# MannLabs/alphadia

Measured on AMD Instinct MI355X. Metric: precursors scored/sec, higher is better.
Workload: dtype f32/f64; 1 GPU; 1000000-precursor predicted library x 3 candidates vs 2h synthetic Thermo-style DIA run (4800 cycles x 61 spectra); BASELINE configs[2] on one GPU; precursors_total=1000000, candidates_total=3000000, candidates_per_gpu=3000000, cycles=4800, parallelism=single GPU, rccl_ranks_seen=1, priming_steps_before_warmup=4

## Files before the change

### alphadia_amd/_abi.py

```python

from __future__ import annotations

import ctypes as C

import numpy as np

NUM_FEATURES = 46
FLAG_SKIP = 1

_f32p = C.POINTER(C.c_float)
_f64p = C.POINTER(C.c_double)
_i64p = C.POINTER(C.c_int64)
_u32p = C.POINTER(C.c_uint32)
_u8p = C.POINTER(C.c_uint8)


class AlphaRaw(C.Structure):
    _fields_ = [
        ("cycle", _f64p),
        ("cycle_len", C.c_int32),
        ("cycle_scans", C.c_int32),
        ("rt_values", _f32p),
        ("n_spectra", C.c_int64),
        ("mobility_values", _f32p),
# ... 123 lines not shown
        ("fragment_precursor_idx", _u32p),
        ("fragment_rank", _u8p),
        ("fragment_mz_library", _f32p),
        ("fragment_mz", _f32p),
        ("fragment_mz_observed", _f32p),
        ("fragment_height", _f32p),
        ("fragment_intensity", _f32p),
        ("fragment_mass_error", _f32p),
        ("fragment_correlation", _f32p),
        ("fragment_position", _u8p),
        ("fragment_number", _u8p),
        ("fragment_type", _u8p),
        ("fragment_charge", _u8p),
        ("fragment_loss_type", _u8p),
    ]


COMPACT_ROW_FIELDS = [("row", np.uint32), ("precursor_idx", np.uint32), ("rank", np.uint8)]
COMPACT_SLOT_FIELDS = [
    ("fragment_row", np.uint32), ("fragment_precursor_idx", np.uint32), ("fragment_rank", np.uint8),
    ("fragment_mz_library", np.float32), ("fragment_mz", np.float32), ("fragment_mz_observed", np.float32),
    ("fragment_height", np.float32), ("fragment_intensity", np.float32), ("fragment_mass_error", np.float32),
    ("fragment_correlation", np.float32), ("fragment_position", np.uint8), ("fragment_number", np.uint8),
    ("fragment_type", np.uint8), ("fragment_charge", np.uint8), ("fragment_loss_type", np.uint8),
]


OUTPUT_FIELDS = [
    ("valid", np.uint8, 1),
    ("precursor_idx", np.uint32, 1),
# ... 568 lines not shown
    "adh_calibrate_staged_fragments": [C.c_void_p, C.POINTER(LoessModel), C.POINTER(C.c_double)],
    "adh_stage_fragments_columns": [C.c_void_p, C.POINTER(Fragments), C.POINTER(LoessModel), C.POINTER(C.c_double)],
    "adh_staged_fragments_read": [C.c_void_p, C.c_int32, C.c_void_p, C.c_int64],
}


N_PLAN_CLASSES = 37
N_GENERIC_GROUPS = 3
PLAN_PROTOTYPES = {
    "adh_plan_class_counts": [C.c_void_p, C.POINTER(C.c_int64), C.c_int32],
    "adh_generic_launch_stats": [C.c_void_p, C.POINTER(C.c_int64), C.c_int32],
}


def declare(lib) -> None:
    for name, argtypes in {**RESIDENT_PROTOTYPES, **STAGE_PART_PROTOTYPES, **APPEND_PROTOTYPES, **QUANT_PROTOTYPES,
                           **PG_PROTOTYPES, **PFDR_PROTOTYPES, **TL_PROTOTYPES, **MBR_PROTOTYPES, **STAGE_LIB_PROTOTYPES, **PLAN_PROTOTYPES}.items():
        fn = getattr(lib, name)
        fn.argtypes = argtypes
        fn.restype = C.c_int
```

### alphadia_amd/csrc/adh_copyout.hip

```cpp

__global__ void adh_slot_count_kernel(const uint16_t *__restrict__ lib_slot, int64_t row0, int64_t n, int top_k,
                                      uint32_t *__restrict__ cnt) {
    const int64_t i = (int64_t)blockIdx.x * blockDim.x + threadIdx.x;
    if (i > n) return;
    uint32_t k = 0;
    if (i < n) {
        const uint16_t *s = lib_slot + (row0 + i) * (int64_t)top_k;
        while (k < (uint32_t)top_k && s[k]) ++k;
    }
    cnt[i] = k;
}

#include "adh_fill_host.h"

struct PadLayout {
    size_t per_row, total;
    PadLayout(int64_t n, int top_k, int64_t n_chunks)
        : per_row(4 + (size_t)top_k * 22), total(base(n, n_chunks + 1, 4 + (size_t)top_k * 22) + 64) {}
    size_t base(int64_t a, int64_t ci) const { return base(a, ci, per_row); }
    static size_t base(int64_t a, int64_t ci, size_t per_row_) {
        return ((size_t)a * per_row_ + ((size_t)(a / kAnchorRows) + (size_t)ci) * 8 + (size_t)ci * 1024 + 255) & ~(size_t)255;
    }
};

__global__ void adh_pad_pack_kernel(DevOut t, int64_t row0, int64_t n, int top_k, unsigned char *__restrict__ block,
                                    uint32_t *__restrict__ total) {
    const int64_t id = (int64_t)blockIdx.x * blockDim.x + threadIdx.x;
    const uint32_t *off = reinterpret_cast<const uint32_t *>(block);
// ... 165 lines not shown
        const uint32_t a = (uint32_t)o, k = (uint32_t)o1 - a;
        if ((uint32_t)s >= k) continue;
        const int64_t r = row0 + i, src = r * (int64_t)top_k + s;
        const size_t dst = (size_t)a + (size_t)s;
        s_slot[dst] = t.fragment_lib_slot[src];
        reinterpret_cast<float *>(block + L.s_f[0])[dst] = t.fragment_mz_observed[src];
        reinterpret_cast<float *>(block + L.s_f[1])[dst] = t.fragment_height[src];
        reinterpret_cast<float *>(block + L.s_f[2])[dst] = t.fragment_intensity[src];
        reinterpret_cast<float *>(block + L.s_f[3])[dst] = t.fragment_mass_error[src];
        reinterpret_cast<float *>(block + L.s_f[4])[dst] = t.fragment_correlation[src];
    }
}

namespace {
void cop_copy_stripe(const unsigned char *block, int64_t cnt_r, int64_t cnt_s, int64_t base_r, int64_t base_s,
                     adh_compact_output_t *out, int w, int T, const adh_candidates_t *c, const LibRec *lib) {
    const CopBlock L((uint64_t)cnt_r, (uint64_t)cnt_s);
    const int64_t lo = cnt_r * w / T, hi = cnt_r * (w + 1) / T;
    if (hi <= lo) return;
    const uint32_t *rows = reinterpret_cast<const uint32_t *>(block + L.row);
    const uint8_t *cnt = block + L.cnt;
    int64_t s_lo = 0;
    for (int64_t j = 0; j < lo; ++j) s_lo += cnt[j];
    memcpy(out->row + base_r + lo, rows + lo, (size_t)(hi - lo) * 4);
    const float *fb = reinterpret_cast<const float *>(block + L.feat);
    for (int k = 0; k < ADH_NUM_FEATURES; ++k)
        memcpy(out->features + (size_t)k * (size_t)out->rows_capacity + (size_t)(base_r + lo),
               fb + (size_t)k * (size_t)cnt_r + (size_t)lo, (size_t)(hi - lo) * 4);
    const uint16_t *slot = reinterpret_cast<const uint16_t *>(block + L.s_slot);
    int64_t d = base_s + s_lo, at = s_lo;
    for (int64_t j = lo; j < hi; ++j) {
        const uint32_t r = rows[j];
        const uint32_t p = c->precursor_idx[r];
        const uint8_t rk = c->rank ? c->rank[r] : (uint8_t)0;
        out->precursor_idx[base_r + j] = p;
        out->rank[base_r + j] = rk;
        const LibRec *base = lib + c->frag_start_idx[r];
        const int k = (int)cnt[j];
        for (int q = 0; q < k; ++q, ++d, ++at) {
            const LibRec &l = base[slot[at] - 1];
            out->fragment_row[d] = r;
            out->fragment_precursor_idx[d] = p;
            out->fragment_rank[d] = rk;
            out->fragment_mz_library[d] = l.mz_library;
            out->fragment_mz[d] = l.mz;
            out->fragment_position[d] = l.position;
// ... 540 lines not shown
        if (!handoff.wait_for(n_chunks - 1))
            return fail(ADH_ERR_HIP, std::string("scoring pipeline (compacted copy-out): ") + hipGetErrorString(handoff.error));
        for (int64_t ci = 0; ci < n_chunks; ++ci) stripe(ci, T);
        team.join_all();
        if (trace.timing)
            fprintf(stderr, "[adh]   compacted copy-out: host team done %.2f ms after the call began (%d threads)\n", trace.since(), T);
        if (trace.timing && sparse)
            fprintf(stderr, "[adh]   sparse-slot wire: %llu filled slots, %llu intensity words and %llu correlation words sent\n",
                    (unsigned long long)wire_slots, (unsigned long long)wire_nz_i, (unsigned long long)wire_nz_c);
        return ADH_OK;
    }
};

struct OperatorCopyOut : CopyOut {
    adh_compact_output_t *const cop;
    const CopLayout lay;
    const int T;
    int started = 0;
    unsigned char *dev_blocks = nullptr, *stage = nullptr;
    std::vector<int64_t> base_r, base_s, cnt_r, cnt_s;
    bool overflow = false;
    BlockHandoff handoff;
    HandoffTeam team{handoff};
    OperatorCopyOut(const CopyOut &call, adh_compact_output_t *cop_)
        : CopyOut(call), cop(cop_), lay(n, top_k, n_chunks), T(host_threads_for(n)), base_r((size_t)n_chunks + 1, 0),
          base_s((size_t)n_chunks + 1, 0), cnt_r((size_t)n_chunks, 0), cnt_s((size_t)n_chunks, 0),
          handoff(n_chunks, h->device) {}

    void advise_huge_pages() const {
        auto advise = [](void *p, size_t bytes) {
            const uintptr_t lo = ((uintptr_t)p + (2u << 20) - 1) & ~(uintptr_t)((2u << 20) - 1);
            const uintptr_t hi = ((uintptr_t)p + bytes) & ~(uintptr_t)((2u << 20) - 1);
            if (hi > lo) (void)madvise((void *)lo, hi - lo, MADV_HUGEPAGE);
        };
        const size_t rc_ = (size_t)cop->rows_capacity, sc_ = (size_t)cop->slots_capacity;
        advise(cop->features, rc_ * ADH_NUM_FEATURES * 4);
        advise(cop->row, rc_ * 4), advise(cop->precursor_idx, rc_ * 4);
        void *const s4[] = {cop->fragment_row, cop->fragment_precursor_idx, cop->fragment_mz_library, cop->fragment_mz,
                            cop->fragment_mz_observed, cop->fragment_height, cop->fragment_intensity,
                            cop->fragment_mass_error, cop->fragment_correlation};
        for (void *p4 : s4) advise(p4, sc_ * 4);
        void *const s1[] = {cop->fragment_rank, cop->fragment_position, cop->fragment_number, cop->fragment_type,
                            cop->fragment_charge, cop->fragment_loss_type};
        for (void *p1 : s1) advise(p1, sc_);
    }
    int prepare() override {
        if (!compact_output_complete(cop)) return fail(ADH_ERR_INVALID_ARGUMENT, "compact output buffer is NULL");
        advise_huge_pages();
        const size_t cnt_bytes = (size_t)(n + n_chunks) * 8;
        int rc = grow_device(&h->cop_cnt, &h->cop_cnt_bytes, cnt_bytes, cnt_bytes / 8);
        if (rc == ADH_OK) rc = grow_scan_scratch<uint64_t>(&h->cop_scan, &h->cop_scan_bytes, longest_chunk() + 1, h->stream);
        if (rc == ADH_OK) rc = grow_pinned(&h->cop_stage, &h->cop_stage_bytes, lay.total, lay.total / 8);
        if (rc != ADH_OK) return rc;
        if (n_chunks > 4096) return fail(ADH_ERR_UNSUPPORTED, "compact output: more than 4096 chunks");
        if (!h->cop_tot_pinned) HIP_TRY(hipHostMalloc((void **)&h->cop_tot_pinned, 4096 * 8, hipHostMallocDefault));
        rc = grow_device(&h->cop_dev, &h->cop_dev_bytes, lay.total, lay.total / 8 + 4096);
        if (rc != ADH_OK) return rc;
        stage = static_cast<unsigned char *>(h->cop_stage), dev_blocks = static_cast<unsigned char *>(h->cop_dev);
        handoff.landed = [this](int64_t ci) {
            const uint64_t tot = h->cop_tot_pinned[ci];
            base_r[(size_t)ci + 1] = base_r[(size_t)ci] + (int64_t)(tot >> 32);
            base_s[(size_t)ci + 1] = base_s[(size_t)ci] + (int64_t)(tot & 0xFFFFFFFFull);
            if (base_r[(size_t)ci + 1] > cop->rows_capacity || base_s[(size_t)ci + 1] > cop->slots_capacity)
                overflow = true;
            cnt_r[(size_t)ci] = overflow ? 0 : (int64_t)(tot >> 32);
            cnt_s[(size_t)ci] = overflow ? 0 : (int64_t)(tot & 0xFFFFFFFFull);
            if (trace.timing)
                fprintf(stderr, "[adh]   compact chunk %lld: %lld rows, %lld slots on the host %.2f ms after the call began\n",
                        (long long)ci, (long long)(tot >> 32), (long long)(tot & 0xFFFFFFFFull), trace.since());
        };
        return ADH_OK;
    }
    void stripe(int64_t ci, int w) {
        if (cnt_r[(size_t)ci] == 0 && cnt_s[(size_t)ci] == 0) return;
        cop_copy_stripe(stage + lay.base(cut[(size_t)ci], ci), cnt_r[(size_t)ci], cnt_s[(size_t)ci], base_r[(size_t)ci],
                        base_s[(size_t)ci], cop, w, T, c, h->h_lib.data());
    }
    void start_team() override {
        started = start_handoff_team(team, T, n_chunks, [this](int64_t ci, int w) { stripe(ci, w); });
    }
    int pack(int64_t ci) override {
        const int64_t a = cut[(size_t)ci], nr = cut[(size_t)ci + 1] - a;
        hipStream_t sk = h->stream;
        uint64_t *off = static_cast<uint64_t *>(h->cop_cnt) + a + ci;
        hipLaunchKernelGGL(adh_cop_count_kernel, dim3((unsigned)((nr + 256) / 256)), dim3(256), 0, sk, dev.valid,
                           dev.fragment_lib_slot, a, nr, top_k, off);
        size_t scan_bytes = h->cop_scan_bytes;
        HIP_TRY(hipcub::DeviceScan::ExclusiveSum(h->cop_scan, scan_bytes, off, off, (int)(nr + 1), sk));
        hipLaunchKernelGGL(adh_cop_pack_kernel, dim3((unsigned)std::min<int64_t>((nr * top_k + 255) / 256, 8192)), dim3(256), 0,
                           sk, dev, h->cs.d, h->d_lib, a, nr, top_k, off, dev_blocks + lay.base(a, ci), h->cop_tot_pinned + ci);
        HIP_TRY(hipGetLastError());
// ... 9 lines not shown
    }
    int copy_out(int64_t ci) override {
        return ci > 0 ? send(ci - 1) : ADH_OK;
    }
    int flush() override { return send(n_chunks - 1); }
    int finish() override {
        if (!handoff.wait_for(n_chunks - 1))
            return fail(ADH_ERR_HIP, std::string("scoring pipeline (compact copy-out): ") + hipGetErrorString(handoff.error));
        team.join_all();
        for (int64_t ci = 0; ci < n_chunks; ++ci)
            for (int w = started; w < T; ++w) stripe(ci, w);
        if (trace.timing)
            fprintf(stderr, "[adh]   compact: host team done %.2f ms after the call began (%d threads)\n", trace.since(), T);
        cop->n_rows = base_r[(size_t)n_chunks];
        cop->n_slots = base_s[(size_t)n_chunks];
        if (overflow) {
            (void)hipStreamSynchronize(h->stream);
            (void)hipStreamSynchronize(h->stream_out);
            tables_stand = true;
            return fail(ADH_ERR_INVALID_ARGUMENT, "compact output: rows_capacity / slots_capacity too small (n_rows / n_slots say what is needed)");
        }
        return ADH_OK;
    }
};

}
```

### alphadia_amd/csrc/adh_score_host.hip

```cpp

namespace {

int comm_wait_slot(adh_handle *h, int slot);
int comm_gather_slot(adh_handle *h, int slot);

struct OutFieldDesc {
    const char *name;
    size_t member;
    int per_row;
    int elem;
    bool wire;
    bool optional;
};

const OutFieldDesc kOutFields[] = {
    {"valid", offsetof(adh_output_t, valid), 1, 1, true, false},
    {"features", offsetof(adh_output_t, features), ADH_NUM_FEATURES, 4, true, false},
    {"fragment_mz_observed", offsetof(adh_output_t, fragment_mz_observed), -1, 4, true, false},
    {"fragment_height", offsetof(adh_output_t, fragment_height), -1, 4, true, false},
    {"fragment_intensity", offsetof(adh_output_t, fragment_intensity), -1, 4, true, false},
    {"fragment_mass_error", offsetof(adh_output_t, fragment_mass_error), -1, 4, true, false},
    {"fragment_correlation", offsetof(adh_output_t, fragment_correlation), -1, 4, true, false},
    {"fragment_lib_slot", offsetof(adh_output_t, fragment_lib_slot), -1, 2, true, true},
    {"precursor_idx", offsetof(adh_output_t, precursor_idx), 1, 4, false, false},
// ... 1056 lines not shown
        for (std::vector<hipEvent_t> *list : {&events, &aux}) {
            h->free_events.insert(h->free_events.end(), list->begin(), list->end());
            list->clear();
        }
        if (!ok) {
            (void)hipDeviceSynchronize();
            (void)hipGetLastError();
            h->last_tables = -1;
            h->last_rows = 0;
            tab.partial = false;
        }
    }
};

int score_pipeline(adh_handle_t *h, const adh_candidates_t *c, const adh_scoring_config_t *cfg, adh_output_t *out,
                   adh_compact_output_t *cop, bool resident = false) {
    if (!h || !c || !cfg || !out) return fail(ADH_ERR_INVALID_ARGUMENT, "NULL argument");
    if (out->n != c->n) return fail(ADH_ERR_INVALID_ARGUMENT, "output rows != candidates");
    int rc = check_candidate_args(h, c);
    if (rc == ADH_OK) rc = check_score_args(h, cfg, out);
    if (rc != ADH_OK) return rc;
    for (int i = 0; i < kNumOutFields && !cop && !resident; ++i)
        if (!kOutFields[i].optional && *out_member(out, kOutFields[i]) == nullptr)
            return fail(ADH_ERR_INVALID_ARGUMENT, "output buffer is NULL");
    HIP_TRY(hipSetDevice(h->device));
    PipelineTrace trace;
    const int64_t n = c->n;
    const int top_k = out->top_k;
    h->plan = Plan();
    h->cands_uploaded = false;
    h->acc_live = false;
// ... 45 lines not shown
    }
    const std::vector<int64_t> cut = chunk_cuts(n, h->tims_staged, max_rows, compact_wanted);
    const int64_t n_chunks = (int64_t)cut.size() - 1;
    const bool compact = compact_wanted && n_chunks <= 4096;
    adh_output_t dev_k = dev;
    if ((rebuild || cop || resident) && !getenv("ADH_DEBUG_WRITE_ALL")) {
        for (int i = 0; i < kNumOutFields; ++i) {
            const OutFieldDesc &f = kOutFields[i];
            if (!f.wire && f.member != offsetof(adh_output_t, stat_matched_peaks)) *out_member(&dev_k, f) = nullptr;
        }
        tab.partial = true;
    }
    const CopyOut call(h, c, dev, cut, chunk_done, tot_ready, trace);
    std::unique_ptr<CopyOut> copy_out;
    if (resident) copy_out.reset(new CopyOut(call));
    else if (cop) copy_out.reset(new OperatorCopyOut(call, cop));
    else if (compact) copy_out.reset(new PackedCopyOut(call, out));
    else copy_out.reset(new PlainCopyOut(call, out, rebuild));
    rc = copy_out->prepare();
    if (rc != ADH_OK) return rc;
    trace.t_1 = trace.now();
    trace.mark_start(si);
    rc = cand_upload_range(h, c, 0, cut[1], si);
    if (rc == ADH_OK) rc = plan_enqueue(h, h->slots[0], cfg, 0, cut[1], si);
    if (rc == ADH_OK && n_chunks > 1) rc = cand_upload_range(h, c, cut[1], cut[2], si);
    if (rc != ADH_OK) return rc;
    copy_out->start_team();
    for (int64_t ci = 0; ci < n_chunks; ++ci) {
        const int64_t a = cut[(size_t)ci], b = cut[(size_t)ci + 1];
        const int ps = (int)(ci & 1);
        if (ci + 1 < n_chunks) {
// ... 30 lines not shown
    if (e != hipSuccess) return fail(ADH_ERR_HIP, std::string("scoring pipeline: ") + hipGetErrorString(e));
    trace.report(cut, chunk_done, compact);
    unwind.ok = true;
    h->tables_current = true;
    return ADH_OK;
}
}

int adh_score_candidates(adh_handle_t *h, const adh_candidates_t *c, const adh_scoring_config_t *cfg,
                         adh_output_t *out) {
    return score_pipeline(h, c, cfg, out, nullptr);
}

int adh_score_candidates_compact(adh_handle_t *h, const adh_candidates_t *c, const adh_scoring_config_t *cfg,
                                 adh_compact_output_t *cop) {
    if (!h || !c || !cfg || !cop) return fail(ADH_ERR_INVALID_ARGUMENT, "NULL argument");
    if (cop->top_k <= 0 || cop->rows_capacity < 0 || cop->slots_capacity < 0)
        return fail(ADH_ERR_INVALID_ARGUMENT, "compact output: top_k / capacities");
    if (cop->top_k > 255)
        return fail(ADH_ERR_INVALID_ARGUMENT, "compact output: top_k above 255");
    if (h->h_lib.size() != (size_t)h->n_lib)
        return fail(ADH_ERR_NOT_STAGED, "compact output: no host copy of the staged library");
    adh_output_t shape{};
    shape.n = c->n;
    shape.top_k = cop->top_k;
    return score_pipeline(h, c, cfg, &shape, cop);
}

int adh_table_layout(int64_t rows, int32_t top_k, int32_t capacity, adh_table_field_t *fields, int32_t *n_fields,
                     uint64_t *total_bytes, uint64_t *wire_bytes) {
    if (rows < 0 || top_k <= 0 || !n_fields) return fail(ADH_ERR_INVALID_ARGUMENT, "adh_table_layout: bad argument");
    *n_fields = kNumOutFields;
    size_t wire = 0;
    const size_t total = layout_tables(nullptr, rows, top_k, nullptr, &wire);
    if (total_bytes) *total_bytes = total;
    if (wire_bytes) *wire_bytes = wire;
    if (!fields) return ADH_OK;
    if (capacity < kNumOutFields) return fail(ADH_ERR_INVALID_ARGUMENT, "adh_table_layout: field array too short");
    size_t off = 0;
    for (int i = 0; i < kNumOutFields; ++i) {
        const OutFieldDesc &f = kOutFields[i];
// ... 278 lines not shown
```

### alphadia_amd/runtime.py

```python

from __future__ import annotations

import ctypes as C
import os

import numpy as np

from alphadia_amd import _abi

_HERE = os.path.dirname(os.path.abspath(__file__))
LIB_PATH = os.environ.get("ADH_LIB_PATH") or os.path.join(_HERE, "libalphadia_hip.so")

EXPORTED_SYMBOLS = [
    "adh_last_error",
    "adh_device_count",
    "adh_create",
    "adh_destroy",
    "adh_stage_alpharaw",
    "adh_stage_timstof",
    "adh_stage_fragments",
    "adh_score_candidates",
    "adh_score_candidates_compact",
    "adh_host_take_objects",
    "adh_trim_device_cache",
    "adh_host_threads",
    "adh_chunk_cuts",
    "adh_upload_candidates",
    "adh_score_uploaded",
    "adh_get_stream",
    "adh_synchronize",
    "adh_kernel_time_ms",
    "adh_fragcomp",
    "adh_fragcomp_stats",
    "adh_fragcomp_frames",
    "adh_select_candidates",
    "adh_select_time_ms",
    "adh_transpose_timstof",
# ... 106 lines not shown


_PROCESS_T0 = _process_start_time()


def _attempt_lower_bound() -> float:
    if os.environ.get("ADH_RUN_NONCE"):
        return _PROCESS_T0 - float(os.environ.get("ADH_RENDEZVOUS_STAGGER_S", "600"))
    return min(_process_start_time(os.getppid()), _PROCESS_T0)


class HipBackendError(RuntimeError):
    pass


def _load():
    if not os.path.exists(LIB_PATH):
        raise ImportError(
            f"{LIB_PATH} not found: build it with `python -c 'import __graft_entry__ as g; "
            "g.build()'` (hipcc --offload-arch=gfx950). There is no CPU fallback."
        )
    lib = C.CDLL(LIB_PATH)
    lib.adh_last_error.restype = C.c_char_p
    for name in EXPORTED_SYMBOLS[1:]:
        getattr(lib, name).restype = C.c_int
    _abi.declare(lib)
    return lib


lib = _load()
# ... 572 lines not shown
        if self.comm_world > 1:
            width = int(round(self.all_reduce_max(float(width))))
        m_out, arrays = _abi.alloc_output(n, width,
                                          with_stats=with_stats, zero=False, alloc=alloc,
                                          with_slots=with_stats or not reuse_buffers)
        cfg = _abi.pack_config(cfg_jit)
        self.tables_serial += 1
        _check(
            lib.adh_score_candidates(self._h, cands.ref(), C.byref(cfg), m_out.ref()),
            "adh_score_candidates",
        )
        self.n_candidates = n
        return arrays

    def score_host_compact(self, cands: _abi.Marshalled, cfg_jit, slots_per_row: float | None = None,
                           buffers: dict | None = None) -> dict:
        n = int(cands.struct.n)
        width = _abi.output_width(cands, int(cfg_jit.top_k_fragments))
        cfg = _abi.pack_config(cfg_jit)
        rows_cap = max(n, 1)
        slots_cap = max(int(n * (width if slots_per_row is None else min(float(slots_per_row), width))) + 1, 1)
        self.tables_serial += 1
        while True:
            out = _abi.CompactOutput()
            out.rows_capacity, out.slots_capacity, out.top_k = rows_cap, slots_cap, width
            key = (rows_cap, slots_cap)
            arrays = buffers.get(key) if buffers is not None else None
            if arrays is None:
                arrays = {}
                for name, dt in _abi.COMPACT_ROW_FIELDS:
                    arrays[name] = np.empty(rows_cap, dtype=dt)
                arrays["features"] = np.empty((_abi.NUM_FEATURES, rows_cap), dtype=np.float32)
                for name, dt in _abi.COMPACT_SLOT_FIELDS:
                    arrays[name] = np.empty(slots_cap, dtype=dt)
                if buffers is not None:
                    buffers.clear()
                    buffers[key] = arrays
            for name, a in arrays.items():
                setattr(out, name, a.ctypes.data_as(dict(out._fields_)[name]))
            rc = lib.adh_score_candidates_compact(self._h, cands.ref(), C.byref(cfg), C.byref(out))
            if rc != 0 and (int(out.n_rows) > rows_cap or int(out.n_slots) > slots_cap):
                rows_cap, slots_cap = max(rows_cap, int(out.n_rows)), max(slots_cap, int(out.n_slots))
                continue
            _check(rc, "adh_score_candidates_compact")
            break
        self.n_candidates = n
        nr, ns = int(out.n_rows), int(out.n_slots)
        res = {name: arrays[name][:nr] for name, _ in _abi.COMPACT_ROW_FIELDS}
        res["features"] = arrays["features"][:, :nr]
        res.update({name: arrays[name][:ns] for name, _ in _abi.COMPACT_SLOT_FIELDS})
        res["top_k"] = width
        return res

    def score_resident(self, cands: _abi.Marshalled, cfg_jit) -> int:
        n = int(cands.struct.n)
        cfg = _abi.pack_config(cfg_jit)
        self.tables_serial += 1
        _check(lib.adh_score_candidates_resident(self._h, cands.ref(), C.byref(cfg)), "adh_score_candidates_resident")
        self.n_candidates = n
        return _abi.output_width(cands, int(cfg_jit.top_k_fragments))

    def score_resident_append(self, cands: _abi.Marshalled, cfg_jit) -> tuple[int, int]:
        cfg = _abi.pack_config(cfg_jit)
        first = C.c_int64(0)
        self.tables_serial += 1
        _check(lib.adh_score_candidates_resident_append(self._h, cands.ref(), C.byref(cfg), C.byref(first)),
               "adh_score_candidates_resident_append")
# ... 907 lines not shown
```

### alphadia_amd/scoring.py

```python

from __future__ import annotations

import logging
import os
from types import SimpleNamespace

import numpy as np
import pandas as pd

from alphadia_amd import _abi

logger = logging.getLogger(__name__)

DEFAULT_FEATURE_COLUMNS = [
    "base_width_mobility",
    "base_width_rt",
    "rt_observed",
    "mobility_observed",
    "mono_ms1_intensity",
    "top_ms1_intensity",
    "sum_ms1_intensity",
    "weighted_ms1_intensity",
    "weighted_mass_deviation",
    "weighted_mass_error",
# ... 480 lines not shown
    cuts = np.linspace(0, n, parts + 1).astype(np.int64)
    found = _parallel([(lambda a=a, b=b: np.flatnonzero(mask_source[a:b] > 0) + a) for a, b in zip(cuts[:-1], cuts[1:])])
    return np.concatenate(found)


def _take_missing_columns(left_df, right_df, right_columns, rows):
    missing = [c for c in dict.fromkeys(right_columns) if c not in left_df.columns]
    absent = [c for c in missing if c not in right_df.columns]
    if absent:
        raise ValueError(f"Columns {absent} must be present in right_df")
    for c in missing:
        left_df[c] = right_df[c].values[rows]
    return left_df


def collect_candidates(
    candidates_df: pd.DataFrame,
    psm_proto_df: OutputPsmDF,
    precursors_flat_df: pd.DataFrame,
    rt_column: str,
    mobility_column: str,
    precursor_mz_column: str,
    row_maps=None,
    sequence_counts=None,
    compact: dict | None = None,
) -> pd.DataFrame:
    candidate_columns = DEFAULT_CANDIDATE_COLUMNS.copy()
    candidate_columns += ["score"] if "score" in candidates_df.columns else []
    if "rank" not in candidates_df.columns:
        candidates_df = candidates_df.assign(rank=np.zeros(len(candidates_df), dtype=np.uint8))
    precursor_df_columns = DEFAULT_PRECURSOR_COLUMNS + get_isotope_column_names(
        precursors_flat_df.columns
    )
    for col in [rt_column, mobility_column, precursor_mz_column]:
        if col not in precursor_df_columns:
            precursor_df_columns.append(col)
    if row_maps is not None:
        return _collect_candidates_by_rows(candidates_df, psm_proto_df, precursors_flat_df, rt_column, candidate_columns,
                                           precursor_df_columns, row_maps, sequence_counts, compact=compact)
    precursor_idx, rank, features = psm_proto_df.to_precursor_df()
    df = pd.DataFrame(features, columns=DEFAULT_FEATURE_COLUMNS)
    df["precursor_idx"] = precursor_idx
    df["rank"] = rank
    df = merge_missing_columns(
        df, candidates_df, candidate_columns, on=["precursor_idx", "rank"], how="left"
    )
    df = merge_missing_columns(
        df, precursors_flat_df, precursor_df_columns, on=["precursor_idx"], how="left"
    )
    df["delta_rt"] = df["rt_observed"] - df[rt_column]
    df["n_K"] = df["sequence"].str.count("K")
    df["n_R"] = df["sequence"].str.count("R")
    df["n_P"] = df["sequence"].str.count("P")
    return df


def _collect_candidates_by_rows(candidates_df, psm_proto_df, precursors_flat_df, rt_column, candidate_columns,
                                precursor_df_columns, row_maps, sequence_counts, compact: dict | None = None) -> pd.DataFrame:
    _, threads = _host_pool()
    rows = compact["row"] if compact is not None else np.flatnonzero(np.asarray(psm_proto_df.valid, dtype=bool))
    cand_rows = np.asarray(row_maps[0]).take(rows)
    prec_rows = np.asarray(row_maps[1]).take(rows)
    names: list[str] = list(DEFAULT_FEATURE_COLUMNS)
    jobs: list[tuple[str, np.ndarray, np.ndarray]] = [] if compact is not None else [
        ("precursor_idx", psm_proto_df.precursor_idx, rows), ("rank", psm_proto_df.rank, rows)]
    have = set(names) | {"precursor_idx", "rank"}
    for frame, wanted, idx in ((candidates_df, candidate_columns, cand_rows),
                               (precursors_flat_df, precursor_df_columns, prec_rows)):
        missing = [c for c in dict.fromkeys(wanted) if c not in have]
        absent = [c for c in missing if c not in frame.columns]
        if absent:
            raise ValueError(f"Columns {absent} must be present in right_df")
        for c in missing:
            jobs.append((c, frame[c].values, idx))
            have.add(c)
    counts = None
    if sequence_counts is not None:
        counts = [(name, np.asarray(cnt), prec_rows) for name, cnt in zip(("n_K", "n_R", "n_P"), sequence_counts, strict=True)]
    if compact is not None:
        features = compact["features"]
    else:
        features = _take_rows_transposed(psm_proto_df.features, rows, threads)
    obj_jobs = [(name, src, idx) for name, src, idx in jobs if src.dtype == object]
    num_jobs = [(name, src, idx) for name, src, idx in jobs if src.dtype != object] + (counts or [])
    from . import runtime as _rt

    pool, n_pool = _host_pool()
    tasks = [(lambda src=src, idx=idx: src[idx]) for _, src, idx in num_jobs]
    futures = [pool.submit(t) for t in tasks] if n_pool > 1 else None
    cols = {}
    for name, src, idx in obj_jobs:
        cols[name] = _rt.take_objects(src, idx, threads)
    gathered = [f.result() for f in futures] if futures is not None else [t() for t in tasks]
    cols.update({name: arr for (name, _, _), arr in zip(num_jobs, gathered)})
    frame = {name: features[j] for j, name in enumerate(DEFAULT_FEATURE_COLUMNS)}
    if compact is not None:
        frame["precursor_idx"] = compact["precursor_idx"]
        frame["rank"] = compact["rank"]
    frame.update({name: cols[name] for name, _, _ in jobs})
    frame["delta_rt"] = frame["rt_observed"] - frame[rt_column]
    if counts is not None:
        for name, _, _ in counts:
            frame[name] = cols[name]
    df = pd.DataFrame(frame, copy=False)
    if counts is None:
        df["n_K"] = df["sequence"].str.count("K")
        df["n_R"] = df["sequence"].str.count("R")
        df["n_P"] = df["sequence"].str.count("P")
    return df


def collect_fragments_compact(compact: dict, precursors_flat_df: pd.DataFrame, prec_rows) -> pd.DataFrame:
    missing = [c for c in ("elution_group_idx", "decoy") if c not in FRAGMENT_DF_COLUMNS]
    absent = [c for c in missing if c not in precursors_flat_df.columns]
    if absent:
        raise ValueError(f"Columns {absent} must be present in right_df")
    _, threads = _host_pool()
    frow = compact["fragment_row"]
    prec_rows = np.asarray(prec_rows)
    lib_rows = np.empty(len(frow), dtype=prec_rows.dtype)
    cuts = np.linspace(0, len(frow), (threads if len(frow) > 1 << 20 else 1) + 1).astype(np.int64)
    _parallel([(lambda a=int(a), b=int(b): np.take(prec_rows, frow[a:b], out=lib_rows[a:b])) for a, b in zip(cuts[:-1], cuts[1:])])
    looked_up = [_take_chunked(precursors_flat_df[c].values, lib_rows, threads) for c in missing]
    frame = {c: compact["fragment_" + c] for c in FRAGMENT_DF_COLUMNS}
    frame.update(dict(zip(missing, looked_up, strict=True)))
    return pd.DataFrame(frame, copy=False)


def collect_fragments(psm_proto_df: OutputPsmDF, precursors_flat_df: pd.DataFrame, prec_rows=None) -> pd.DataFrame:
    if prec_rows is None:
        idx = psm_proto_df.fragment_rows()
        df = pd.DataFrame(dict(zip(FRAGMENT_DF_COLUMNS, psm_proto_df.to_fragment_df(idx), strict=True)))
        return merge_missing_columns(
            df, precursors_flat_df, ["elution_group_idx", "decoy"], on=["precursor_idx"], how="left"
        )
    _, threads = _host_pool()
    top_k = psm_proto_df.fragment_mz_library.shape[1]
    idx = _flatnonzero_chunked(psm_proto_df.fragment_mz_library.reshape(-1), threads)
# ... 149 lines not shown
        if "exc" in frag_box:
            raise frag_box["exc"]
        fragments_df = frag_box["df"]
        t_4 = time.perf_counter()
        self.last_timings = {"assemble_ms": (t_1 - t_0) * 1e3, "score_ms": (t_2 - t_1) * 1e3,
                             "collect_candidates_ms": (t_3 - t_2) * 1e3, "collect_fragments_ms": frag_box["ms"],
                             "collect_ms": (t_4 - t_2) * 1e3, "total_ms": (t_4 - t_0) * 1e3}
        logger.info("Finished candidate scoring")
        return features_df, fragments_df


def _call_compact(self, candidates_df: pd.DataFrame, soa: dict, t_0: float, t_1: float):
    import threading
    import time

    comp = self._ctx.score_host_compact(pack_assembled(soa), self._kernel_config())
    t_2 = time.perf_counter()
    frag_box: dict = {}

    def fragments_job():
        t_a = time.perf_counter()
        try:
            frag_box["df"] = collect_fragments_compact(comp, self.precursors_flat_df, soa["prec_row"])
        except BaseException as exc:
            frag_box["exc"] = exc
        frag_box["ms"] = (time.perf_counter() - t_a) * 1e3

    logger.info("Collecting candidate and fragment features")
    worker = threading.Thread(target=fragments_job, name="adh-collect-fragments")
    worker.start()
    try:
# ... 2 lines not shown
            row_maps=(soa["order"], soa["prec_row"]), sequence_counts=self._sequence_counts(), compact=comp)
    finally:
        t_3 = time.perf_counter()
        worker.join()
    if "exc" in frag_box:
        raise frag_box["exc"]
    t_4 = time.perf_counter()
    self.last_timings = {"assemble_ms": (t_1 - t_0) * 1e3, "score_ms": (t_2 - t_1) * 1e3,
                         "collect_candidates_ms": (t_3 - t_2) * 1e3, "collect_fragments_ms": frag_box["ms"],
                         "collect_ms": (t_4 - t_2) * 1e3, "total_ms": (t_4 - t_0) * 1e3,
                         "wire_bytes": int(comp["features"].nbytes + 5 * len(comp["row"]) + 22 * len(comp["fragment_row"]))}
    logger.info("Finished candidate scoring")
    return features_df, frag_box["df"]


HipCandidateScoring._call_compact = _call_compact


class ResidentScores:

    def __init__(self, scorer: "HipCandidateScoring", candidates_df: pd.DataFrame, soa: dict, serial: int):
        self._scorer = scorer
        self._candidates_df = candidates_df
        self._serial = serial
        self.order = soa["order"]
        self.prec_row = soa["prec_row"]
        self.metadata = pd.DataFrame({name: np.asarray(soa[name]) for name in
                                      ("precursor_idx", "rank", "decoy", "elution_group_idx", "channel")})
        self._columns = None

    @property
# ... 278 lines not shown
```

### include/alphadia_hip.h

```cpp
#ifndef ALPHADIA_HIP_H
#define ALPHADIA_HIP_H

#include <stdint.h>

#ifdef __cplusplus
extern "C" {
#endif

#define ADH_OK 0
#define ADH_ERR_INVALID_ARGUMENT (-1)
#define ADH_ERR_HIP (-2)
#define ADH_ERR_NOT_STAGED (-3)
#define ADH_ERR_UNSUPPORTED (-4)
#define ADH_ERR_OUT_OF_MEMORY (-5)

#define ADH_NUM_FEATURES 46

#define ADH_FLAG_SKIP 1u

typedef struct adh_alpharaw {
    const double *cycle;
    int32_t cycle_len;
    int32_t cycle_scans;
    const float *rt_values;
// ... 134 lines not shown
    float *fragment_mz_observed;
    float *fragment_height;
    float *fragment_intensity;
    float *fragment_mass_error;
    float *fragment_correlation;
    uint8_t *fragment_position;
    uint8_t *fragment_number;
    uint8_t *fragment_type;
    uint8_t *fragment_charge;
    uint8_t *fragment_loss_type;
} adh_compact_output_t;

int adh_score_candidates_compact(adh_handle_t *handle, const adh_candidates_t *candidates,
                                 const adh_scoring_config_t *config, adh_compact_output_t *out);

int adh_upload_candidates(adh_handle_t *handle, const adh_candidates_t *candidates);
int adh_score_uploaded(adh_handle_t *handle, const adh_scoring_config_t *config,
                       adh_output_t *out_device, void *hip_stream);

int adh_get_device_tables(adh_handle_t *handle, adh_output_t *device_view);

int adh_score_candidates_resident(adh_handle_t *handle, const adh_candidates_t *candidates,
                                  const adh_scoring_config_t *config);

int adh_take_rows(adh_handle_t *handle, const int64_t *rows, int64_t n, adh_compact_output_t *out);

int adh_score_candidates_resident_append(adh_handle_t *handle, const adh_candidates_t *candidates,
                                         const adh_scoring_config_t *config, int64_t *first_row);

int adh_resident_reset(adh_handle_t *handle);
// ... 305 lines not shown
```

Before: 54.11 million precursors/s.

## Gather candidate and precursor metadata columns inside native compact copy-out

Adds a source-column interface so the native host copy-out threads gather candidate-, precursor- and per-fragment metadata columns (such as elution_group_idx and decoy) in tiles while they write the compact output. The Python collection step can then skip its separate row-map takes and numpy gathers for those columns. This folds a post-scoring host pass into the already parallel, pipelined copy-out and removes extra passes over the result arrays. In exchange it adds bounds checks, more copy-out work per chunk and a larger ABI surface.

```diff
diff --git a/alphadia_amd/_abi.py b/alphadia_amd/_abi.py
--- a/alphadia_amd/_abi.py
+++ b/alphadia_amd/_abi.py
@@ -161,6 +161,36 @@
         ("fragment_charge", _u8p),
         ("fragment_loss_type", _u8p),
     ]
+
+
+class SourceColumn(C.Structure):
+
+    _fields_ = [
+        ("src", C.c_void_p),
+        ("dst", C.c_void_p),
+        ("n_src", C.c_int64),
+        ("elem_bytes", C.c_int32),
+        ("index", C.c_int32),
+        ("per_slot", C.c_int32),
+        ("reserved", C.c_int32),
+    ]
+
+
+class SourceColumns(C.Structure):
+
+    _fields_ = [
+        ("n_columns", C.c_int64),
+        ("columns", C.POINTER(SourceColumn)),
+        ("candidate_row", C.POINTER(C.c_int64)),
+        ("precursor_row", C.POINTER(C.c_int64)),
+    ]
+
+
+SRC_TABLE_ROW, SRC_CANDIDATE_ROW, SRC_PRECURSOR_ROW = 0, 1, 2
+SOURCE_PROTOTYPES = {
+    "adh_score_candidates_compact_src": [C.c_void_p, C.c_void_p, C.c_void_p, C.POINTER(CompactOutput),
+                                         C.POINTER(SourceColumns)],
+}
 
 
 COMPACT_ROW_FIELDS = [("row", np.uint32), ("precursor_idx", np.uint32), ("rank", np.uint8)]
@@ -759,7 +789,7 @@
 
 
 def declare(lib) -> None:
-    for name, argtypes in {**RESIDENT_PROTOTYPES, **STAGE_PART_PROTOTYPES, **APPEND_PROTOTYPES, **QUANT_PROTOTYPES,
+    for name, argtypes in {**SOURCE_PROTOTYPES, **RESIDENT_PROTOTYPES, **STAGE_PART_PROTOTYPES, **APPEND_PROTOTYPES, **QUANT_PROTOTYPES,
                            **PG_PROTOTYPES, **PFDR_PROTOTYPES, **TL_PROTOTYPES, **MBR_PROTOTYPES, **STAGE_LIB_PROTOTYPES, **PLAN_PROTOTYPES}.items():
         fn = getattr(lib, name)
         fn.argtypes = argtypes
diff --git a/alphadia_amd/csrc/adh_copyout.hip b/alphadia_amd/csrc/adh_copyout.hip
--- a/alphadia_amd/csrc/adh_copyout.hip
+++ b/alphadia_amd/csrc/adh_copyout.hip
@@ -12,6 +12,7 @@
 }
 
 #include "adh_fill_host.h"
+#include "adh_source_cols.h"
 
 struct PadLayout {
     size_t per_row, total;
@@ -207,7 +208,8 @@
 
 namespace {
 void cop_copy_stripe(const unsigned char *block, int64_t cnt_r, int64_t cnt_s, int64_t base_r, int64_t base_s,
-                     adh_compact_output_t *out, int w, int T, const adh_candidates_t *c, const LibRec *lib) {
+                     adh_compact_output_t *out, int w, int T, const adh_candidates_t *c, const LibRec *lib,
+                     const SrcPlan *src = nullptr) {
     const CopBlock L((uint64_t)cnt_r, (uint64_t)cnt_s);
     const int64_t lo = cnt_r * w / T, hi = cnt_r * (w + 1) / T;
     if (hi <= lo) return;
@@ -222,7 +224,11 @@
                fb + (size_t)k * (size_t)cnt_r + (size_t)lo, (size_t)(hi - lo) * 4);
     const uint16_t *slot = reinterpret_cast<const uint16_t *>(block + L.s_slot);
     int64_t d = base_s + s_lo, at = s_lo;
-    for (int64_t j = lo; j < hi; ++j) {
+    for (int64_t j = lo, tile_end = lo; j < hi; ++j) {
+        if (src && j == tile_end) {
+            tile_end = std::min(hi, j + kSrcTile);
+            src->gather_tile(rows + j, cnt + j, tile_end - j, base_r + j, d);
+        }
         const uint32_t r = rows[j];
         const uint32_t p = c->precursor_idx[r];
         const uint8_t rk = c->rank ? c->rank[r] : (uint8_t)0;
@@ -793,6 +799,8 @@
 
 struct OperatorCopyOut : CopyOut {
     adh_compact_output_t *const cop;
+    const adh_source_columns_t *const sources;
+    SrcPlan src;
     const CopLayout lay;
     const int T;
     int started = 0;
@@ -801,8 +809,8 @@
     bool overflow = false;
     BlockHandoff handoff;
     HandoffTeam team{handoff};
-    OperatorCopyOut(const CopyOut &call, adh_compact_output_t *cop_)
-        : CopyOut(call), cop(cop_), lay(n, top_k, n_chunks), T(host_threads_for(n)), base_r((size_t)n_chunks + 1, 0),
+    OperatorCopyOut(const CopyOut &call, adh_compact_output_t *cop_, const adh_source_columns_t *sources_)
+        : CopyOut(call), cop(cop_), sources(sources_), lay(n, top_k, n_chunks), T(host_threads_for(n)), base_r((size_t)n_chunks + 1, 0),
           base_s((size_t)n_chunks + 1, 0), cnt_r((size_t)n_chunks, 0), cnt_s((size_t)n_chunks, 0),
           handoff(n_chunks, h->device) {}
 
@@ -822,9 +830,14 @@
         void *const s1[] = {cop->fragment_rank, cop->fragment_position, cop->fragment_number, cop->fragment_type,
                             cop->fragment_charge, cop->fragment_loss_type};
         for (void *p1 : s1) advise(p1, sc_);
+        for (int k = 0; k < 3; ++k) {
+            for (const SrcPlan::Col &col : src.row_cols[k]) advise(col.dst, rc_ * (size_t)col.elem);
+            for (const SrcPlan::Col &col : src.slot_cols[k]) advise(col.dst, sc_ * (size_t)col.elem);
+        }
     }
     int prepare() override {
         if (!compact_output_complete(cop)) return fail(ADH_ERR_INVALID_ARGUMENT, "compact output buffer is NULL");
+        if (const char *wrong = src.build(sources)) return fail(ADH_ERR_INVALID_ARGUMENT, wrong);
         advise_huge_pages();
         const size_t cnt_bytes = (size_t)(n + n_chunks) * 8;
         int rc = grow_device(&h->cop_cnt, &h->cop_cnt_bytes, cnt_bytes, cnt_bytes / 8);
@@ -853,7 +866,7 @@
     void stripe(int64_t ci, int w) {
         if (cnt_r[(size_t)ci] == 0 && cnt_s[(size_t)ci] == 0) return;
         cop_copy_stripe(stage + lay.base(cut[(size_t)ci], ci), cnt_r[(size_t)ci], cnt_s[(size_t)ci], base_r[(size_t)ci],
-                        base_s[(size_t)ci], cop, w, T, c, h->h_lib.data());
+                        base_s[(size_t)ci], cop, w, T, c, h->h_lib.data(), src.empty() ? nullptr : &src);
     }
     void start_team() override {
         started = start_handoff_team(team, T, n_chunks, [this](int64_t ci, int w) { stripe(ci, w); });
@@ -893,6 +906,12 @@
             fprintf(stderr, "[adh]   compact: host team done %.2f ms after the call began (%d threads)\n", trace.since(), T);
         cop->n_rows = base_r[(size_t)n_chunks];
         cop->n_slots = base_s[(size_t)n_chunks];
+        if (src.bad.load(std::memory_order_relaxed) && !overflow) {
+            (void)hipStreamSynchronize(h->stream);
+            (void)hipStreamSynchronize(h->stream_out);
+            tables_stand = true;
+            return fail(ADH_ERR_INVALID_ARGUMENT, "source columns: a row map points outside a source column");
+        }
         if (overflow) {
             (void)hipStreamSynchronize(h->stream);
             (void)hipStreamSynchronize(h->stream_out);
diff --git a/alphadia_amd/csrc/adh_score_host.hip b/alphadia_amd/csrc/adh_score_host.hip
--- a/alphadia_amd/csrc/adh_score_host.hip
+++ b/alphadia_amd/csrc/adh_score_host.hip
@@ -1094,7 +1094,7 @@
 };
 
 int score_pipeline(adh_handle_t *h, const adh_candidates_t *c, const adh_scoring_config_t *cfg, adh_output_t *out,
-                   adh_compact_output_t *cop, bool resident = false) {
+                   adh_compact_output_t *cop, bool resident = false, const adh_source_columns_t *sources = nullptr) {
     if (!h || !c || !cfg || !out) return fail(ADH_ERR_INVALID_ARGUMENT, "NULL argument");
     if (out->n != c->n) return fail(ADH_ERR_INVALID_ARGUMENT, "output rows != candidates");
     int rc = check_candidate_args(h, c);
@@ -1170,7 +1170,7 @@
     const CopyOut call(h, c, dev, cut, chunk_done, tot_ready, trace);
     std::unique_ptr<CopyOut> copy_out;
     if (resident) copy_out.reset(new CopyOut(call));
-    else if (cop) copy_out.reset(new OperatorCopyOut(call, cop));
+    else if (cop) copy_out.reset(new OperatorCopyOut(call, cop, sources));
     else if (compact) copy_out.reset(new PackedCopyOut(call, out));
     else copy_out.reset(new PlainCopyOut(call, out, rebuild));
     rc = copy_out->prepare();
@@ -1231,6 +1231,11 @@
 
 int adh_score_candidates_compact(adh_handle_t *h, const adh_candidates_t *c, const adh_scoring_config_t *cfg,
                                  adh_compact_output_t *cop) {
+    return adh_score_candidates_compact_src(h, c, cfg, cop, nullptr);
+}
+
+int adh_score_candidates_compact_src(adh_handle_t *h, const adh_candidates_t *c, const adh_scoring_config_t *cfg,
+                                     adh_compact_output_t *cop, const adh_source_columns_t *sources) {
     if (!h || !c || !cfg || !cop) return fail(ADH_ERR_INVALID_ARGUMENT, "NULL argument");
     if (cop->top_k <= 0 || cop->rows_capacity < 0 || cop->slots_capacity < 0)
         return fail(ADH_ERR_INVALID_ARGUMENT, "compact output: top_k / capacities");
@@ -1241,7 +1246,7 @@
     adh_output_t shape{};
     shape.n = c->n;
     shape.top_k = cop->top_k;
-    return score_pipeline(h, c, cfg, &shape, cop);
+    return score_pipeline(h, c, cfg, &shape, cop, false, sources);
 }
 
 int adh_table_layout(int64_t rows, int32_t top_k, int32_t capacity, adh_table_field_t *fields, int32_t *n_fields,
diff --git a/alphadia_amd/csrc/adh_source_cols.h b/alphadia_amd/csrc/adh_source_cols.h
--- /dev/null
+++ b/alphadia_amd/csrc/adh_source_cols.h
@@ -0,0 +1,102 @@
+#pragma once
+#include <stdint.h>
+#include <string.h>
+
+#include <atomic>
+#include <vector>
+
+#include "../../include/alphadia_hip.h"
+
+namespace {
+
+constexpr int64_t kSrcTile = 1024;
+
+struct SrcPlan {
+    struct Col {
+        const unsigned char *src;
+        unsigned char *dst;
+        int elem;
+    };
+    std::vector<Col> row_cols[3], slot_cols[3];
+    const int64_t *map[3] = {nullptr, nullptr, nullptr};
+    int64_t least[3] = {0, 0, 0};
+    bool used[3] = {false, false, false};
+    mutable std::atomic<int> bad{0};
+
+    bool empty() const { return !(used[0] || used[1] || used[2]); }
+
+    const char *build(const adh_source_columns_t *s) {
+        if (!s || s->n_columns == 0) return nullptr;
+        if (s->n_columns < 0 || !s->columns) return "source columns: n_columns / columns";
+        map[ADH_SRC_CANDIDATE_ROW] = s->candidate_row, map[ADH_SRC_PRECURSOR_ROW] = s->precursor_row;
+        for (int64_t i = 0; i < s->n_columns; ++i) {
+            const adh_source_column_t &c = s->columns[i];
+            if (c.elem_bytes != 1 && c.elem_bytes != 2 && c.elem_bytes != 4 && c.elem_bytes != 8)
+                return "source columns: elem_bytes must be 1, 2, 4 or 8";
+            if (c.index < ADH_SRC_TABLE_ROW || c.index > ADH_SRC_PRECURSOR_ROW) return "source columns: unknown index kind";
+            if (c.per_slot != 0 && c.per_slot != 1) return "source columns: per_slot must be 0 or 1";
+            if (!c.dst || c.n_src < 0 || (!c.src && c.n_src > 0)) return "source columns: src / dst / n_src";
+            if (c.index != ADH_SRC_TABLE_ROW && !map[c.index]) return "source columns: a column uses a row map that is NULL";
+            least[c.index] = used[c.index] ? (c.n_src < least[c.index] ? c.n_src : least[c.index]) : c.n_src;
+            used[c.index] = true;
+            (c.per_slot ? slot_cols : row_cols)[c.index].push_back(
+                Col{static_cast<const unsigned char *>(c.src), static_cast<unsigned char *>(c.dst), c.elem_bytes});
+        }
+        return nullptr;
+    }
+
+    template <typename W>
+    static void take(const Col &c, const int64_t *idx, int64_t m, int64_t at) {
+        const unsigned char *s = c.src;
+        unsigned char *d = c.dst + (size_t)at * sizeof(W);
+        for (int64_t i = 0; i < m; ++i) {
+            if (idx[i] < 0) continue;
+            W v;
+            memcpy(&v, s + (size_t)idx[i] * sizeof(W), sizeof(W));
+            memcpy(d + (size_t)i * sizeof(W), &v, sizeof(W));
+        }
+    }
+    template <typename W>
+    static void take_slots(const Col &c, const int64_t *idx, const uint8_t *cnt, int64_t m, int64_t at) {
+        const unsigned char *s = c.src;
+        unsigned char *d = c.dst + (size_t)at * sizeof(W);
+        for (int64_t i = 0; i < m; ++i) {
+            const int k = (int)cnt[i];
+            if (idx[i] >= 0 && k) {
+                W v;
+                memcpy(&v, s + (size_t)idx[i] * sizeof(W), sizeof(W));
+                for (int q = 0; q < k; ++q) memcpy(d + (size_t)q * sizeof(W), &v, sizeof(W));
+            }
+            d += (size_t)k * sizeof(W);
+        }
+    }
+    static void take_any(const Col &c, const int64_t *idx, const uint8_t *cnt, int64_t m, int64_t at) {
+        switch (c.elem) {
+            case 1: cnt ? take_slots<uint8_t>(c, idx, cnt, m, at) : take<uint8_t>(c, idx, m, at); break;
+            case 2: cnt ? take_slots<uint16_t>(c, idx, cnt, m, at) : take<uint16_t>(c, idx, m, at); break;
+            case 4: cnt ? take_slots<uint32_t>(c, idx, cnt, m, at) : take<uint32_t>(c, idx, m, at); break;
+            default: cnt ? take_slots<uint64_t>(c, idx, cnt, m, at) : take<uint64_t>(c, idx, m, at); break;
+        }
+    }
+
+    void gather_tile(const uint32_t *rows, const uint8_t *cnt, int64_t m, int64_t out_r, int64_t out_s) const {
+        int64_t idx[kSrcTile];
+        for (int k = 0; k < 3; ++k) {
+            if (!used[k]) continue;
+            const int64_t *const mp = map[k];
+            const uint64_t bound = (uint64_t)least[k];
+            bool out_of_range = false;
+            for (int64_t i = 0; i < m; ++i) {
+                const int64_t v = mp ? mp[rows[i]] : (int64_t)rows[i];
+                const bool ok = (uint64_t)v < bound;
+                out_of_range |= !ok;
+                idx[i] = ok ? v : -1;
+            }
+            if (out_of_range) bad.store(1, std::memory_order_relaxed);
+            for (const Col &c : row_cols[k]) take_any(c, idx, nullptr, m, out_r);
+            for (const Col &c : slot_cols[k]) take_any(c, idx, cnt, m, out_s);
+        }
+    }
+};
+
+}
diff --git a/alphadia_amd/runtime.py b/alphadia_amd/runtime.py
--- a/alphadia_amd/runtime.py
+++ b/alphadia_amd/runtime.py
@@ -21,6 +21,7 @@
     "adh_stage_fragments",
     "adh_score_candidates",
     "adh_score_candidates_compact",
+    "adh_score_candidates_compact_src",
     "adh_host_take_objects",
     "adh_trim_device_cache",
     "adh_host_threads",
@@ -157,6 +158,11 @@
     pass
 
 
+def native_source(src) -> bool:
+    return (isinstance(src, np.ndarray) and src.ndim == 1 and src.dtype.kind in "biufMm" and not src.dtype.hasobject
+            and src.dtype.itemsize in (1, 2, 4, 8) and src.flags.c_contiguous and src.dtype.isnative)
+
+
 def _load():
     if not os.path.exists(LIB_PATH):
         raise ImportError(
@@ -759,7 +765,7 @@
         return arrays
 
     def score_host_compact(self, cands: _abi.Marshalled, cfg_jit, slots_per_row: float | None = None,
-                           buffers: dict | None = None) -> dict:
+                           buffers: dict | None = None, sources: dict | None = None) -> dict:
         n = int(cands.struct.n)
         width = _abi.output_width(cands, int(cfg_jit.top_k_fragments))
         cfg = _abi.pack_config(cfg_jit)
@@ -781,9 +787,16 @@
                 if buffers is not None:
                     buffers.clear()
                     buffers[key] = arrays
+            fields = dict(out._fields_)
             for name, a in arrays.items():
-                setattr(out, name, a.ctypes.data_as(dict(out._fields_)[name]))
-            rc = lib.adh_score_candidates_compact(self._h, cands.ref(), C.byref(cfg), C.byref(out))
+                if name in fields:
+                    setattr(out, name, a.ctypes.data_as(fields[name]))
+            if sources is None:
+                rc = lib.adh_score_candidates_compact(self._h, cands.ref(), C.byref(cfg), C.byref(out))
+            else:
+                desc, keep = self._source_columns(sources, n, rows_cap, slots_cap, arrays)
+                rc = lib.adh_score_candidates_compact_src(self._h, cands.ref(), C.byref(cfg), C.byref(out), C.byref(desc))
+                del keep
             if rc != 0 and (int(out.n_rows) > rows_cap or int(out.n_slots) > slots_cap):
                 rows_cap, slots_cap = max(rows_cap, int(out.n_rows)), max(slots_cap, int(out.n_slots))
                 continue
@@ -795,7 +808,37 @@
         res["features"] = arrays["features"][:, :nr]
         res.update({name: arrays[name][:ns] for name, _ in _abi.COMPACT_SLOT_FIELDS})
         res["top_k"] = width
+        if sources is not None:
+            res["sources"] = {key: arrays[("source", key)][:ns if per_slot else nr]
+                              for key, _, _, per_slot in sources["columns"]}
         return res
+
+    @staticmethod
+    def _source_columns(sources: dict, n: int, rows_cap: int, slots_cap: int, arrays: dict):
+        maps = []
+        for name in ("candidate_row", "precursor_row"):
+            m = sources.get(name)
+            if m is not None:
+                m = np.ascontiguousarray(m, dtype=np.int64)
+                if m.shape != (n,):
+                    raise ValueError(f"sources[{name!r}] must have one entry per candidate")
+            maps.append(m)
+        cols = (_abi.SourceColumn * max(len(sources["columns"]), 1))()
+        for i, (key, src, index, per_slot) in enumerate(sources["columns"]):
+            if not native_source(src):
+                raise ValueError(f"source column {key!r}: not a contiguous 1-D array of 1-, 2-, 4- or 8-byte elements")
+            cap = slots_cap if per_slot else rows_cap
+            dst = arrays.get(("source", key))
+            if dst is None or dst.dtype != src.dtype or len(dst) != cap:
+                dst = arrays[("source", key)] = np.empty(cap, dtype=src.dtype)
+            cols[i].src, cols[i].dst, cols[i].n_src = src.ctypes.data, dst.ctypes.data, len(src)
+            cols[i].elem_bytes, cols[i].index, cols[i].per_slot = src.dtype.itemsize, int(index), int(bool(per_slot))
+        desc = _abi.SourceColumns()
+        desc.n_columns, desc.columns = len(sources["columns"]), cols
+        i64p = C.POINTER(C.c_int64)
+        desc.candidate_row = maps[0].ctypes.data_as(i64p) if maps[0] is not None else None
+        desc.precursor_row = maps[1].ctypes.data_as(i64p) if maps[1] is not None else None
+        return desc, (cols, maps, [src for _, src, _, _ in sources["columns"]])
 
     def score_resident(self, cands: _abi.Marshalled, cfg_jit) -> int:
         n = int(cands.struct.n)
diff --git a/alphadia_amd/scoring.py b/alphadia_amd/scoring.py
--- a/alphadia_amd/scoring.py
+++ b/alphadia_amd/scoring.py
@@ -518,6 +518,37 @@
     return left_df
 
 
+def _frame_columns(candidates_df, precursors_flat_df, rt_column, mobility_column, precursor_mz_column):
+    candidate_columns = DEFAULT_CANDIDATE_COLUMNS.copy()
+    candidate_columns += ["score"] if "score" in candidates_df.columns else []
+    if "rank" not in candidates_df.columns:
+        candidates_df = candidates_df.assign(rank=np.zeros(len(candidates_df), dtype=np.uint8))
+    precursor_df_columns = DEFAULT_PRECURSOR_COLUMNS + get_isotope_column_names(
+        precursors_flat_df.columns
+    )
+    for col in [rt_column, mobility_column, precursor_mz_column]:
+        if col not in precursor_df_columns:
+            precursor_df_columns.append(col)
+    return candidates_df, candidate_columns, precursor_df_columns
+
+
+def _taken_over_columns(candidates_df, precursors_flat_df, candidate_columns, precursor_df_columns, sequence_counts):
+    jobs: list[tuple[str, np.ndarray, int]] = []
+    have = set(DEFAULT_FEATURE_COLUMNS) | {"precursor_idx", "rank"}
+    for which, (frame, wanted) in enumerate(((candidates_df, candidate_columns), (precursors_flat_df, precursor_df_columns))):
+        missing = [c for c in dict.fromkeys(wanted) if c not in have]
+        absent = [c for c in missing if c not in frame.columns]
+        if absent:
+            raise ValueError(f"Columns {absent} must be present in right_df")
+        for c in missing:
+            jobs.append((c, frame[c].values, which))
+            have.add(c)
+    counts = None
+    if sequence_counts is not None:
+        counts = [(name, np.asarray(cnt), 1) for name, cnt in zip(("n_K", "n_R", "n_P"), sequence_counts, strict=True)]
+    return jobs, counts
+
+
 def collect_candidates(
     candidates_df: pd.DataFrame,
     psm_proto_df: OutputPsmDF,
@@ -529,16 +560,8 @@
     sequence_counts=None,
     compact: dict | None = None,
 ) -> pd.DataFrame:
-    candidate_columns = DEFAULT_CANDIDATE_COLUMNS.copy()
-    candidate_columns += ["score"] if "score" in candidates_df.columns else []
-    if "rank" not in candidates_df.columns:
-        candidates_df = candidates_df.assign(rank=np.zeros(len(candidates_df), dtype=np.uint8))
-    precursor_df_columns = DEFAULT_PRECURSOR_COLUMNS + get_isotope_column_names(
-        precursors_flat_df.columns
-    )
-    for col in [rt_column, mobility_column, precursor_mz_column]:
-        if col not in precursor_df_columns:
-            precursor_df_columns.append(col)
+    candidates_df, candidate_columns, precursor_df_columns = _frame_columns(
+        candidates_df, precursors_flat_df, rt_column, mobility_column, precursor_mz_column)
     if row_maps is not None:
         return _collect_candidates_by_rows(candidates_df, psm_proto_df, precursors_flat_df, rt_column, candidate_columns,
                                            precursor_df_columns, row_maps, sequence_counts, compact=compact)
@@ -563,36 +586,28 @@
                                 precursor_df_columns, row_maps, sequence_counts, compact: dict | None = None) -> pd.DataFrame:
     _, threads = _host_pool()
     rows = compact["row"] if compact is not None else np.flatnonzero(np.asarray(psm_proto_df.valid, dtype=bool))
-    cand_rows = np.asarray(row_maps[0]).take(rows)
-    prec_rows = np.asarray(row_maps[1]).take(rows)
-    names: list[str] = list(DEFAULT_FEATURE_COLUMNS)
+    taken = {key[1]: col for key, col in (compact or {}).get("sources", {}).items() if key[0] == "features"}
+    taken_over, counts = _taken_over_columns(candidates_df, precursors_flat_df, candidate_columns, precursor_df_columns,
+                                             sequence_counts)
+    left = {which for name, _, which in taken_over + (counts or []) if name not in taken}
+    maps = [np.asarray(row_maps[which]).take(rows) if which in left else None for which in (0, 1)]
     jobs: list[tuple[str, np.ndarray, np.ndarray]] = [] if compact is not None else [
         ("precursor_idx", psm_proto_df.precursor_idx, rows), ("rank", psm_proto_df.rank, rows)]
-    have = set(names) | {"precursor_idx", "rank"}
-    for frame, wanted, idx in ((candidates_df, candidate_columns, cand_rows),
-                               (precursors_flat_df, precursor_df_columns, prec_rows)):
-        missing = [c for c in dict.fromkeys(wanted) if c not in have]
-        absent = [c for c in missing if c not in frame.columns]
-        if absent:
-            raise ValueError(f"Columns {absent} must be present in right_df")
-        for c in missing:
-            jobs.append((c, frame[c].values, idx))
-            have.add(c)
-    counts = None
-    if sequence_counts is not None:
-        counts = [(name, np.asarray(cnt), prec_rows) for name, cnt in zip(("n_K", "n_R", "n_P"), sequence_counts, strict=True)]
+    jobs += [(name, src, maps[which]) for name, src, which in taken_over]
+    if counts is not None:
+        counts = [(name, src, maps[which]) for name, src, which in counts]
     if compact is not None:
         features = compact["features"]
     else:
         features = _take_rows_transposed(psm_proto_df.features, rows, threads)
-    obj_jobs = [(name, src, idx) for name, src, idx in jobs if src.dtype == object]
-    num_jobs = [(name, src, idx) for name, src, idx in jobs if src.dtype != object] + (counts or [])
+    obj_jobs = [(name, src, idx) for name, src, idx in jobs if src.dtype == object and name not in taken]
+    num_jobs = [(name, src, idx) for name, src, idx in jobs + (counts or []) if src.dtype != object and name not in taken]
     from . import runtime as _rt
 
     pool, n_pool = _host_pool()
     tasks = [(lambda src=src, idx=idx: src[idx]) for _, src, idx in num_jobs]
     futures = [pool.submit(t) for t in tasks] if n_pool > 1 else None
-    cols = {}
+    cols = dict(taken)
     for name, src, idx in obj_jobs:
         cols[name] = _rt.take_objects(src, idx, threads)
     gathered = [f.result() for f in futures] if futures is not None else [t() for t in tasks]
@@ -620,12 +635,16 @@
     if absent:
         raise ValueError(f"Columns {absent} must be present in right_df")
     _, threads = _host_pool()
-    frow = compact["fragment_row"]
-    prec_rows = np.asarray(prec_rows)
-    lib_rows = np.empty(len(frow), dtype=prec_rows.dtype)
-    cuts = np.linspace(0, len(frow), (threads if len(frow) > 1 << 20 else 1) + 1).astype(np.int64)
-    _parallel([(lambda a=int(a), b=int(b): np.take(prec_rows, frow[a:b], out=lib_rows[a:b])) for a, b in zip(cuts[:-1], cuts[1:])])
-    looked_up = [_take_chunked(precursors_flat_df[c].values, lib_rows, threads) for c in missing]
+    taken = {key[1]: col for key, col in compact.get("sources", {}).items() if key[0] == "fragments"}
+    if all(c in taken for c in missing):
+        looked_up = [taken[c] for c in missing]
+    else:
+        frow = compact["fragment_row"]
+        prec_rows = np.asarray(prec_rows)
+        lib_rows = np.empty(len(frow), dtype=prec_rows.dtype)
+        cuts = np.linspace(0, len(frow), (threads if len(frow) > 1 << 20 else 1) + 1).astype(np.int64)
+        _parallel([(lambda a=int(a), b=int(b): np.take(prec_rows, frow[a:b], out=lib_rows[a:b])) for a, b in zip(cuts[:-1], cuts[1:])])
+        looked_up = [taken[c] if c in taken else _take_chunked(precursors_flat_df[c].values, lib_rows, threads) for c in missing]
     frame = {c: compact["fragment_" + c] for c in FRAGMENT_DF_COLUMNS}
     frame.update(dict(zip(missing, looked_up, strict=True)))
     return pd.DataFrame(frame, copy=False)
@@ -805,7 +824,8 @@
     import threading
     import time
 
-    comp = self._ctx.score_host_compact(pack_assembled(soa), self._kernel_config())
+    comp = self._ctx.score_host_compact(pack_assembled(soa), self._kernel_config(),
+                                        sources=self._source_columns(candidates_df, soa))
     t_2 = time.perf_counter()
     frag_box: dict = {}
 
@@ -838,7 +858,26 @@
     return features_df, frag_box["df"]
 
 
+def _source_columns(self, candidates_df: pd.DataFrame, soa: dict) -> dict:
+    from .runtime import native_source
+
+    frame, candidate_columns, precursor_df_columns = _frame_columns(
+        candidates_df, self.precursors_flat_df, self.rt_column, self.mobility_column, self.precursor_mz_column)
+    taken_over, counts = _taken_over_columns(frame, self.precursors_flat_df, candidate_columns, precursor_df_columns,
+                                             self._sequence_counts())
+    kinds = (_abi.SRC_CANDIDATE_ROW, _abi.SRC_PRECURSOR_ROW)
+    columns = [(("features", name), src, kinds[which], False) for name, src, which in taken_over + counts
+               if native_source(src)]
+    for name in ("elution_group_idx", "decoy"):
+        if name not in FRAGMENT_DF_COLUMNS and name in self.precursors_flat_df.columns:
+            src = self.precursors_flat_df[name].values
+            if native_source(src):
+                columns.append((("fragments", name), src, _abi.SRC_PRECURSOR_ROW, True))
+    return {"columns": columns, "candidate_row": soa["order"], "precursor_row": soa["prec_row"]}
+
+
 HipCandidateScoring._call_compact = _call_compact
+HipCandidateScoring._source_columns = _source_columns
 
 
 class ResidentScores:
diff --git a/include/alphadia_hip.h b/include/alphadia_hip.h
--- a/include/alphadia_hip.h
+++ b/include/alphadia_hip.h
@@ -172,6 +172,29 @@
 int adh_score_candidates_compact(adh_handle_t *handle, const adh_candidates_t *candidates,
                                  const adh_scoring_config_t *config, adh_compact_output_t *out);
 
+enum { ADH_SRC_TABLE_ROW = 0, ADH_SRC_CANDIDATE_ROW = 1, ADH_SRC_PRECURSOR_ROW = 2 };
+
+typedef struct adh_source_column {
+    const void *src;
+    void *dst;
+    int64_t n_src;
+    int32_t elem_bytes;
+    int32_t index;
+    int32_t per_slot;
+    int32_t reserved;
+} adh_source_column_t;
+
+typedef struct adh_source_columns {
+    int64_t n_columns;
+    const adh_source_column_t *columns;
+    const int64_t *candidate_row;
+    const int64_t *precursor_row;
+} adh_source_columns_t;
+
+int adh_score_candidates_compact_src(adh_handle_t *handle, const adh_candidates_t *candidates,
+                                     const adh_scoring_config_t *config, adh_compact_output_t *out,
+                                     const adh_source_columns_t *sources);
+
 int adh_upload_candidates(adh_handle_t *handle, const adh_candidates_t *candidates);
 int adh_score_uploaded(adh_handle_t *handle, const adh_scoring_config_t *config,
                        adh_output_t *out_device, void *hip_stream);
```

After: 53.55 million precursors/s, median of 2. Within noise of the previous version (-1.0%).
